# qwopqwop200/GPTQ-for-LLaMa

Hardware: NVIDIA H100
Metric: tokens/sec LLaMA-7B int4 g128 batch=1; matvec HBM GB/s vs 3.35 TB/s roofline (higher is better)
Workload: dtype f16

## Files before the change

### gptq-for-llama_b200/csrc/decode_mega.cu

```cuda
#include <cuda.h>
#include <cudaTypedefs.h>

#include "common.cuh"
#include "int4_core.cuh"
#include "kernels.h"

namespace gptq {
namespace {

using namespace int4;

constexpr int kTeams = 2;
constexpr int kTeamWarps = 8;
constexpr int kTeamThreads = kTeamWarps * 32;
constexpr int kConsumers = kTeams * kTeamThreads;
constexpr int kConsumerWarps = kTeams * kTeamWarps;
constexpr int kBlock = kConsumers + 32 * kTeams;
constexpr int kSlabCols = 256;
constexpr int kStageSteps = 4;
constexpr int kStepBytes = 4096;
constexpr int kScaleOff = kStageSteps * kStepBytes;
constexpr int kZeroOff = kScaleOff + 512;
constexpr int kStageBytes = 17 * 1024;
constexpr int kHD = 128;
// ... 55 lines not shown

struct MatDesc {
    const __half* sc;
    const uint32_t* qz;
    int gs_steps;
    int tmap;
    int chunk0;
};
struct LayerDesc {
    MatDesc qkv, o, gate, up, down;
    const __half* input_norm;
    const __half* post_norm;
    const int32_t* qkv_perm;
    const int32_t* o_perm;
    const int32_t* mlp_perm;
};
constexpr int kMaxTP = 8;
struct MegaParams {
    int n_layers, H, Hq, I, V, v0, v1, n_heads, max_seq, n_stages, lm_rows;
    int tp_size, tp_rank, tp_exchange;
    float eps, inv_base, scale;
    const __half* embed;
    const __half* final_norm;
    const __half* lm_head;
    const int32_t* tokens;
    const int32_t* positions;
    __half* k_cache;
    __half* v_cache;
    size_t layer_stride;
    __half* logits;
    int32_t* next_token;
    __half* resid[2];
    float* acc_qkv;
    float* acc_o;
    float* acc_g;
    float* acc_u;
    float* acc_d;
    float* part;
    float* rope_cs;
    unsigned long long* bar;
    float* acc_o_loc;
    float* acc_d_loc;
    float* acc_o_peer[kMaxTP];
    float* acc_d_peer[kMaxTP];
    __half* logits_peer[kMaxTP];
    unsigned long long* xbar_peer[kMaxTP];
    LayerDesc layers[kMaxLayers];
    CUtensorMap tmaps[6];
    int batch, xs_stride;
};

__device__ __forceinline__ void team_range(unsigned T, unsigned U, unsigned nb, int& a, int& b) {
    a = (int)((T * U) / nb);
    b = (int)(((T + 1) * U) / nb);
}
struct HeadTeams {
    int first, count;
};
__device__ __forceinline__ HeadTeams head_teams(int head, int n_heads, unsigned nb) {
    const int base = (int)nb / n_heads, rem = (int)nb % n_heads;
    HeadTeams h;
    h.first = head * base + min(head, rem);
    h.count = base + (head < rem ? 1 : 0);
    return h;
}
__device__ __forceinline__ void attn_range(unsigned T, int n_heads, unsigned nb, int upb, int& head, int& b0, int& b1) {
    const int base = (int)nb / n_heads, rem = (int)nb % n_heads;
    const int split = rem * (base + 1);
    int idx, cnt;
    if ((int)T < split) {
        head = (int)T / (base + 1);
        idx = (int)T - head * (base + 1);
        cnt = base + 1;
    } else {
        head = rem + ((int)T - split) / base;
        idx = ((int)T - split) % base;
        cnt = base;
// ... 18 lines not shown
    }
    const long long extra = (long long)nb - (long long)p.batch * p.n_heads;
    HeadTeams h;
    h.first = s * p.n_heads + (int)(extra * before / tot);
    h.count = (s + 1) * p.n_heads + (int)(extra * (before + mine) / tot) - h.first;
    return h;
}
__device__ __forceinline__ int team_seq(const MegaParams& p, unsigned T, unsigned nb, HeadTeams& st) {
    int s = 0;
#pragma unroll 1
    for (;; ++s) {
        st = seq_teams(p, s, nb);
        if ((int)T < st.first + st.count || s == p.batch - 1) return s;
    }
}
template <bool BATCH>
__device__ __forceinline__ int attn_work(const MegaParams& p, unsigned T, unsigned nb, int& pos, int& Tlen, int& head, int& b0, int& b1) {
    int s = 0;
    HeadTeams st{0, (int)nb};
    if constexpr (BATCH) {
        s = team_seq(p, T, nb, st);
        pos = step_pos(p, s);
    } else {
        pos = step_pos(p);
    }
    Tlen = pos + 1;
    const int upb = (Tlen + kKeysPerUnit - 1) / kKeysPerUnit;
    attn_range(T - st.first, p.n_heads, st.count, upb, head, b0, b1);
    return s;
}

__device__ __forceinline__ void team_sync(int team) { asm volatile("bar.sync %0, 256;" ::"r"(team + 1) : "memory"); }
__device__ __forceinline__ void cta_sync() { asm volatile("bar.sync 3, 512;" ::: "memory"); }

struct ProdRing {
    uint32_t ring, full, empty;
    int stage, use, nstages;
#ifdef GPTQ_TRACE
    long long blocked;
#endif
};
__device__ __forceinline__ uint32_t prod_acquire(ProdRing& r, uint32_t& bar) {
#ifdef GPTQ_TRACE
    const long long t0 = clock64();
#endif
    if (r.use > 0) mbar_wait_backoff(r.empty + r.stage * 8, (r.use - 1) & 1u);
#ifdef GPTQ_TRACE
    r.blocked += clock64() - t0;
#endif
    bar = r.full + r.stage * 8;
    return r.ring + r.stage * kStageBytes;
}
__device__ __forceinline__ void prod_advance(ProdRing& r) {
    if (++r.stage == r.nstages) {
        r.stage = 0;
        ++r.use;
    }
}

__device__ __forceinline__ void tma_load_3d(uint32_t dst, const CUtensorMap* tm, int c0, int c1, int c2, uint32_t bar) {
    asm volatile("cp.async.bulk.tensor.3d.shared::cluster.global.mbarrier::complete_tx::bytes [%0], [%1, {%2, %3, %4}], [%5];" ::"r"(dst), "l"(tm), "r"(c0),
                 "r"(c1), "r"(c2), "r"(bar)
                 : "memory");
}

template <int NM>
// ... 335 lines not shown
        a[1] = h2_as_u32(__hfma2(nibbles_to_h2<0x00f000f0u>(q), sixteenth, m64));
        a[2] = h2_as_u32(__hsub2(nibbles_to_h2<0x000f000fu>(q8), c1024));
        a[3] = h2_as_u32(__hfma2(nibbles_to_h2<0x00f000f0u>(q8), sixteenth, m64));
    }
}

template <bool FIRST>
__device__ __forceinline__ void step_mma(const uint4& q, const uint4& xf, float (&acc0)[4], float (&acc1)[4]) {
    uint32_t c0[4], c1[4], c2[4], c3[4];
    nibble_regs(q.x, c0);
    nibble_regs(q.y, c1);
    nibble_regs(q.z, c2);
    nibble_regs(q.w, c3);
    if (FIRST) {
        mma_16816_z(acc0, c0[0], c1[0], c0[1], c1[1], xf.x, xf.y);
        mma_16816_z(acc1, c2[0], c3[0], c2[1], c3[1], xf.x, xf.y);
    } else {
        mma_16816(acc0, c0[0], c1[0], c0[1], c1[1], xf.x, xf.y);
        mma_16816(acc1, c2[0], c3[0], c2[1], c3[1], xf.x, xf.y);
    }
    mma_16816(acc0, c0[2], c1[2], c0[3], c1[3], xf.z, xf.w);
    mma_16816(acc1, c2[2], c3[2], c2[3], c3[3], xf.z, xf.w);
}

enum XMode { X_FULL = 0, X_ATTN = 1, X_SWIGLU = 2 };

struct TeamCtx {
    int team, wt, lane, ttid;
    unsigned T, nb;
    __half* xseg;
    float* xsum_seg;
    uint8_t* scratch;
};

template <int NB>
__device__ __forceinline__ float merge_records(const MegaParams& p, const HeadTeams& ht, int d) {
    float M = -INFINITY, Ls = 0.f, O = 0.f;
#pragma unroll 1
    for (int ib = 0; ib < ht.count; ib += NB) {
        float mv[NB], lv[NB], ov[NB];
#pragma unroll
        for (int i = 0; i < NB; ++i) {
            const bool on = ib + i < ht.count;
            const float* rc = p.part + (size_t)(ht.first + (on ? ib + i : 0)) * kRec;
            const float m = ld_cg(rc), l = ld_cg(rc + 1), o = ld_cg(rc + 4 + d);
            mv[i] = on ? m : -INFINITY;
            lv[i] = on ? l : 0.f;
            ov[i] = on ? o : 0.f;
        }
        float Mb = M;
#pragma unroll
        for (int i = 0; i < NB; ++i) Mb = fmaxf(Mb, mv[i]);
        const float w0 = (M == -INFINITY) ? 0.f : expf(M - Mb);
        Ls *= w0;
        O *= w0;
#pragma unroll
        for (int i = 0; i < NB; ++i) {
            const float w = (mv[i] == -INFINITY) ? 0.f : expf(mv[i] - Mb);
            Ls = fmaf(lv[i], w, Ls);
            O = fmaf(ov[i], w, O);
        }
        M = Mb;
    }
    return O / Ls;
}

// ... 147 lines not shown
            const uint32_t o1 = h2_as_u32(__floats2half2_rn(swiglu(g0.z, a0.z), swiglu(g0.w, a0.w)));
            const uint32_t o2 = h2_as_u32(__floats2half2_rn(swiglu(g1.x, a1.x), swiglu(g1.y, a1.y)));
            const uint32_t o3 = h2_as_u32(__floats2half2_rn(swiglu(g1.z, a1.z), swiglu(g1.w, a1.w)));
            *reinterpret_cast<uint4*>(tc.xseg + (size_t)s * p.xs_stride + cs * 8) = perm8(o0, o1, o2, o3);
        }
    } else {
#pragma unroll 1
        for (int s = 0; s < B; ++s) {
            const HeadTeams st = seq_teams(p, s, tc.nb);
            __half* xseg = tc.xseg + (size_t)s * p.xs_stride;
            for (int e = tc.ttid; e < nfeat; e += kTeamThreads) {
                int k = k_of(e);
                if constexpr (ACT) {
                    if (perm != nullptr) k = perm[k];
                }
                const int head = k / kHD, d = k - head * kHD;
                HeadTeams ht = head_teams(head, p.n_heads, st.count);
                ht.first += st.first;
                __half hv = __float2half_rn(merge_records<12>(p, ht, d));
                const int j8 = e & 7;
                if (perm_scaled(j8)) hv = __hmul(hv, __float2half_rn(0.0625f));
                xseg[(e & ~7) + perm_pos(j8)] = hv;
            }
        }
    }
    team_sync(tc.team);
#pragma unroll 1
    for (int s = 0; s < B; ++s) compute_xsum(tc.xseg + (size_t)s * p.xs_stride, nun, tc.xsum_seg + s * (p.H / 32), tc.ttid, kTeamThreads);
    team_sync(tc.team);
}

template <int NM, int XMODE, bool ACT = false, bool BATCH = false>
__device__ void run_matvec(const MegaParams& p, ConsRing& ring, const TeamCtx& tc, int gs_steps, int K, int N, float* out0, float* out1, const __half* xs_full,
                           const float* xsum_full, const int32_t* perm = nullptr, float* const* peers = nullptr) {
    const int lane = tc.lane, g = lane >> 2, t = lane & 3;
    const int nk = K / 32, nslab = N / kSlabCols;
    int u, u_end;
    team_range(tc.T, (unsigned)(NM * nslab) * nk, tc.nb, u, u_end);
    const int cg = (g >> 1) | ((g & 1) << 2);
    const int col_l = 4 * cg + t;
    const uint32_t lane_a0 = (uint32_t)((tc.wt * 16 + t) * 128 + ((cg ^ t) * 16));
    const uint32_t lane_a1 = (uint32_t)((tc.wt * 16 + t) * 128 + ((cg ^ t ^ 4) * 16));
    const uint32_t lane_b = (uint32_t)((tc.wt * 4 + t) * 128 + ((cg ^ (4 * (tc.wt & 1) + t)) * 16));
    const uint32_t lane_s = (uint32_t)(kScaleOff + (tc.wt * 32 + col_l) * 2);
    const uint32_t lane_z = (uint32_t)(kZeroOff + (tc.wt * 4 + (cg >> 1)) * 4);
    const int zshift = (cg & 1) * 16 + t * 4;
    const float unit = kSubnormal ? 16777216.0f : 1.0f;
    const int B = p.batch;
    const int xsum_hi = BATCH ? (min(2 * t + 1, B - 1) - min(2 * t, B - 1)) * (p.H / 32) : 0;
    const int u_begin = u;
    if constexpr (XMODE != X_FULL) {
        if (u < u_end) {
#ifdef GPTQ_TRACE
            const long long stg0 = clock64();
#endif
            if constexpr (BATCH)
                stage_range_batch<XMODE, ACT>(p, tc, nk, u, u_end, perm);
            else
                stage_range<XMODE, ACT>(p, tc, nk, u, u_end, perm);
#ifdef GPTQ_TRACE
            if (g_mega_trace != nullptr && threadIdx.x == 0) g_mega_trace[blockIdx.x * 64 + 36 + XMODE] += (unsigned long long)(clock64() - stg0);
#endif
        }
    }

#pragma unroll 1
    while (u < u_end) {
// ... 70 lines not shown
                }
            } else {
                uint32_t sh, zw;
                asm volatile("ld.shared.u16 %0, [%1];" : "=r"(sh) : "r"(st + lane_s));
                asm volatile("ld.shared.u32 %0, [%1];" : "=r"(zw) : "r"(st + lane_z));
                const float a = (t & 2) ? ((t & 1) ? acc1[2] : acc1[0]) : ((t & 1) ? acc0[2] : acc0[0]);
                const float z = (float)(((zw >> zshift) & 15u) + 1u);
                tot = fmaf(__half2float(__ushort_as_half((unsigned short)sh)), fmaf(a, unit, -z * xs4), tot);
            }
            cons_release(ring, lane);
            xaddr += n * 64;
            xsum += n;
            left -= n;
            gpos += n;
            if (gpos == gs_steps) gpos = 0;
        }
        if constexpr (BATCH) {
            float* outq = (mi ? out1 : out0) + (slab_v - mi * nslab) * kSlabCols + tc.wt * 32 + 4 * cg;
#pragma unroll
            for (int j = 0; j < 2; ++j) {
                if (2 * t + j < B)
                    asm volatile("red.global.add.v4.f32 [%0], {%1, %2, %3, %4};" ::"l"(outq + (size_t)(2 * t + j) * N), "f"(totb[0][j]), "f"(totb[1][j]),
                                 "f"(totb[2][j]), "f"(totb[3][j])
                                 : "memory");
            }
        } else if (peers == nullptr) {
            asm volatile("red.global.add.f32 [%0], %1;" ::"l"(outp), "f"(tot) : "memory");
        } else {
            const size_t off = (size_t)(outp - out0);
            for (int q = 0; q < p.tp_size; ++q) asm volatile("red.relaxed.sys.global.add.f32 [%0], %1;" ::"l"(peers[q] + off), "f"(tot) : "memory");
        }
        u += nseg;
    }
}

template <bool BATCH>
__device__ void run_attention(const MegaParams& p, ConsRing& ring, const TeamCtx& tc, int layer) {
    int pos, Tlen, head, b0, b_end;
    const int seq = attn_work<BATCH>(p, tc.T, tc.nb, pos, Tlen, head, b0, b_end);
    float* red_o = reinterpret_cast<float*>(tc.scratch);
    float* red_ml = reinterpret_cast<float*>(tc.scratch + 4096);
    float* q_s = reinterpret_cast<float*>(tc.scratch);
    __half* knew = reinterpret_cast<__half*>(tc.scratch + 512);
    __half* vnew = knew + kHD;
    const int ttid = tc.ttid, lane = tc.lane, grp = ttid >> 3, j = ttid & 7;
    const int ub_new = pos / kKeysPerUnit;
    __half* kc_l = p.k_cache + layer * p.layer_stride;
    __half* vc_l = p.v_cache + layer * p.layer_stride;
    float* rec = p.part + (size_t)tc.T * kRec;
    if (b0 >= b_end) {
        if (ttid < kHD) rec[4 + ttid] = 0.f;
        if (ttid == 0) {
            rec[0] = -INFINITY;
            rec[1] = 0.f;
        }
        return;
    }
    {
        const int nseg = b_end - b0;
        const bool owns_new = (ub_new >= b0 && ub_new < b_end);
        team_sync(tc.team);
        if (ttid < kHD) {
            const int i = ttid & 63;
            const bool hi = ttid >= 64;
            const float c = ld_cg(p.rope_cs + seq * kHD + i), s = ld_cg(p.rope_cs + seq * kHD + 64 + i);
            const float* aq = p.acc_qkv + (size_t)seq * 3 * p.Hq + head * kHD;
            const float qx = __half2float(__float2half_rn(ld_cg(aq + i))), qy = __half2float(__float2half_rn(ld_cg(aq + i + 64)));
            const float qr = hi ? __fadd_rn(__fmul_rn(qx, s), __fmul_rn(qy, c)) : __fsub_rn(__fmul_rn(qx, c), __fmul_rn(qy, s));
            q_s[ttid] = __half2float(__float2half_rn(qr));
            if (owns_new) {
                const float* ak = aq + p.Hq;
                const float* av = aq + 2 * p.Hq;
                const float kx = __half2float(__float2half_rn(ld_cg(ak + i))), ky = __half2float(__float2half_rn(ld_cg(ak + i + 64)));
                const float kr = hi ? __fadd_rn(__fmul_rn(kx, s), __fmul_rn(ky, c)) : __fsub_rn(__fmul_rn(kx, c), __fmul_rn(ky, s));
                const __half kh = __float2half_rn(kr), vh = __float2half_rn(ld_cg(av + ttid));
                knew[ttid] = kh;
                vnew[ttid] = vh;
                const size_t off = ((size_t)(seq * p.n_heads + head) * p.max_seq + pos) * kHD + ttid;
                kc_l[off] = kh;
                vc_l[off] = vh;
            }
        }
        team_sync(tc.team);
        float qr[16];
#pragma unroll
        for (int d = 0; d < 8; ++d) {
            qr[d] = q_s[8 * j + d];
            qr[8 + d] = q_s[64 + 8 * j + d];
        }
        float mloc = -INFINITY, lloc = 0.f, o[16];
#pragma unroll
        for (int d = 0; d < 16; ++d) o[d] = 0.f;
#pragma unroll 1
        for (int b = b0; b < b0 + nseg; ++b) {
            const uint32_t st = cons_wait(ring);
            if (b == ub_new) {
                team_sync(tc.team);
                const int row = pos - b * kKeysPerUnit;
// ... 55 lines not shown
            mloc = mn;
        }
        if (lane < 8) {
            if (lane == 0) {
                red_ml[tc.wt * 2] = mloc;
                red_ml[tc.wt * 2 + 1] = lloc;
            }
#pragma unroll
            for (int d = 0; d < 8; ++d) {
                red_o[tc.wt * kHD + 8 * lane + d] = o[d];
                red_o[tc.wt * kHD + 64 + 8 * lane + d] = o[8 + d];
            }
        }
        team_sync(tc.team);
        if (ttid < kHD) {
            float M = -INFINITY;
#pragma unroll
            for (int w = 0; w < kTeamWarps; ++w) M = fmaxf(M, red_ml[w * 2]);
            float L = 0.f, O = 0.f;
#pragma unroll
            for (int w = 0; w < kTeamWarps; ++w) {
                const float mw = red_ml[w * 2];
                const float wgt = (mw == -INFINITY) ? 0.f : expf(mw - M);
                L = fmaf(red_ml[w * 2 + 1], wgt, L);
                O = fmaf(red_o[w * kHD + ttid], wgt, O);
            }
            rec[4 + ttid] = O;
            if (ttid == 0) {
                rec[0] = M;
                rec[1] = L;
            }
        }
    }
}

__device__ void run_lm_head(const MegaParams& p, ConsRing& ring, const TeamCtx& tc, const __half* xs_plain) {
    const int R = p.lm_rows, H = p.H, nch = H / 8;
    int u, u_end;
    const int nloc = p.v1 - p.v0;
    team_range(tc.T, (unsigned)((nloc + R - 1) / R), tc.nb, u, u_end);
    float* part_s = reinterpret_cast<float*>(tc.scratch);
    float xr[4][8];
#pragma unroll
    for (int i = 0; i < 4; ++i) {
        const int c = tc.ttid + i * kTeamThreads;
        if (c < nch) {
            const uint4 v = *reinterpret_cast<const uint4*>(xs_plain + c * 8);
            const uint32_t w[4] = {v.x, v.y, v.z, v.w};
#pragma unroll
            for (int e = 0; e < 4; ++e) {
                const float2 f = __half22float2(u32_as_h2(w[e]));
                xr[i][2 * e] = f.x;
                xr[i][2 * e + 1] = f.y;
            }
        } else {
#pragma unroll
            for (int e = 0; e < 8; ++e) xr[i][e] = 0.f;
        }
    }
    int buf = 0;
#pragma unroll 1
    for (; u < u_end; ++u) {
        const int nrows = min(R, nloc - u * R);
        const uint32_t st = cons_wait(ring);
        float* ps = part_s + buf * (R * kTeamWarps);
#pragma unroll 1
// ... 178 lines not shown
    ConsRing ring;
    ring.ring = smem_u32(smem_raw) + tc.team * ring_bytes;
    ring.full = smem_u32(&bars_s[tc.team][0]);
    ring.tile = ring.ring;
    ring.bar = ring.full;
    ring.parity = 0;
    ring.left = p.n_stages;
    ring.nstages = p.n_stages;
#ifdef GPTQ_TRACE
    ring.waited = 0;
    ring.stages = 0;
#endif

    unsigned long long gen;
    {
        unsigned long long v;
        asm volatile("ld.acquire.gpu.global.u64 %0, [%1];" : "=l"(v) : "l"(p.bar + 1) : "memory");
        gen = v;
    }
    unsigned long long xgen = 0;
    if (p.tp_size > 1) asm volatile("ld.acquire.sys.global.u64 %0, [%1];" : "=l"(xgen) : "l"(p.xbar_peer[p.tp_rank] + 32 * kMaxTP) : "memory");
    auto sync_all_ranks = [&](float* loc, float* const* peers) {
        if (p.tp_size == 1) {
            grid_barrier(p.bar, gen);
        } else {
            if (p.tp_exchange && loc != nullptr) {
                grid_barrier(p.bar, gen);
                tp_exchange(p, loc, peers, p.H);
            }
            tp_barrier(p, xgen);
        }
    };

    if constexpr (BATCH) {
        if (blockIdx.x == 0 && tid < 64 * nbat) {
            const int s = tid >> 6, i = tid & 63;
            const float f = expf((float)i * p.inv_base) * (float)step_pos(p, s);
            p.rope_cs[s * kHD + i] = cosf(f);
            p.rope_cs[s * kHD + 64 + i] = sinf(f);
        }
    } else if (blockIdx.x == 0 && tid < 64) {
        const float f = expf((float)tid * p.inv_base) * (float)step_pos(p);
        p.rope_cs[tid] = cosf(f);
        p.rope_cs[64 + tid] = sinf(f);
    }

    const int token = min(max(p.tokens[0], 0), p.V - 1);
    const __half* resid_src = p.embed + (size_t)token * p.H;
    const float* resid_acc = nullptr;
    int cur = 1;
    auto stage_norms = [&](bool plain, const __half* src, const float* acc, const __half* norm_w, __half* resid_out, const int32_t* perm) {
#pragma unroll 1
        for (int s = 0; s < nbat; ++s) {
            const __half* src_s = acc != nullptr ? src + (size_t)s * p.H : p.embed + (size_t)min(max(p.tokens[s], 0), p.V - 1) * p.H;
            const float* acc_s = acc != nullptr ? acc + (size_t)s * p.H : nullptr;
            __half* out_s = resid_out != nullptr ? resid_out + (size_t)s * p.H : nullptr;
            if (plain)
                stage_norm<false, true>(p, src_s, acc_s, norm_w, out_s, xs + (size_t)s * p.xs_stride, xsum + s * (p.H / 32), tmp, red_s, nullptr);
            else
                stage_norm<ACT, false>(p, src_s, acc_s, norm_w, out_s, xs + (size_t)s * p.xs_stride, xsum + s * (p.H / 32), tmp, red_s, perm);
        }
    };
#pragma unroll 1
    for (int l = 0; l < p.n_layers; ++l) {
        const LayerDesc& L = p.layers[l];
        MTRACE(l * 12 + 0);
        if constexpr (BATCH)
            stage_norms(false, resid_src, resid_acc, L.input_norm, p.resid[cur ^ 1], L.qkv_perm);
        else
            stage_norm<ACT, false>(p, resid_src, resid_acc, L.input_norm, p.resid[cur ^ 1], xs, xsum, tmp, red_s, L.qkv_perm);
        MTRACE(l * 12 + 1);
        cur ^= 1;
        zero_slice(p.acc_g, nbat * p.I);
        zero_slice(p.acc_u, nbat * p.I);
        {
            OPTRACE_BEGIN(ring);
            run_matvec<1, X_FULL, false, BATCH>(p, ring, tc, L.qkv.gs_steps, p.H, 3 * p.Hq, p.acc_qkv, nullptr, xs, xsum);
            OPTRACE_END(ring, l, 0);
        }
        MTRACE(l * 12 + 2);
        grid_barrier(p.bar, gen);
        MTRACE(l * 12 + 3);
        zero_slice(p.acc_d, nbat * p.H);
        {
            OPTRACE_BEGIN(ring);
            run_attention<BATCH>(p, ring, tc, l);
            OPTRACE_END(ring, l, 1);
        }
        MTRACE(l * 12 + 4);
        grid_barrier(p.bar, gen);
        MTRACE(l * 12 + 5);
        zero_slice(p.acc_qkv, nbat * 3 * p.Hq);
        {
            OPTRACE_BEGIN(ring);
            if constexpr (BATCH)
                run_matvec<1, X_ATTN, ACT, true>(p, ring, tc, L.o.gs_steps, p.Hq, p.H, p.acc_o, nullptr, xs, xsum, L.o_perm);
            else
                run_matvec<1, X_ATTN, ACT>(p, ring, tc, L.o.gs_steps, p.Hq, p.H, p.tp_exchange ? p.acc_o_loc : p.acc_o, nullptr, xs, xsum, L.o_perm, (p.tp_size > 1 && !p.tp_exchange) ? p.acc_o_peer : nullptr);
            OPTRACE_END(ring, l, 2);
        }
        MTRACE(l * 12 + 6);
        sync_all_ranks(p.acc_o_loc, p.acc_o_peer);
        MTRACE(l * 12 + 7);
        if constexpr (BATCH)
            stage_norms(false, p.resid[cur], p.acc_o, L.post_norm, p.resid[cur ^ 1], L.mlp_perm);
        else
            stage_norm<ACT, false>(p, p.resid[cur], p.acc_o, L.post_norm, p.resid[cur ^ 1], xs, xsum, tmp, red_s, L.mlp_perm);
        cur ^= 1;
        MTRACE(l * 12 + 8);
        {
            OPTRACE_BEGIN(ring);
            run_matvec<2, X_FULL, false, BATCH>(p, ring, tc, L.gate.gs_steps, p.H, p.I, p.acc_g, p.acc_u, xs, xsum);
            OPTRACE_END(ring, l, 3);
        }
        MTRACE(l * 12 + 9);
        grid_barrier(p.bar, gen);
        zero_slice(p.acc_o, nbat * p.H);
        MTRACE(l * 12 + 10);
        {
            OPTRACE_BEGIN(ring);
            if constexpr (BATCH)
                run_matvec<1, X_SWIGLU, false, true>(p, ring, tc, L.down.gs_steps, p.I, p.H, p.acc_d, nullptr, xs, xsum);
            else
                run_matvec<1, X_SWIGLU>(p, ring, tc, L.down.gs_steps, p.I, p.H, p.tp_exchange ? p.acc_d_loc : p.acc_d, nullptr, xs, xsum, nullptr, (p.tp_size > 1 && !p.tp_exchange) ? p.acc_d_peer : nullptr);
            OPTRACE_END(ring, l, 4);
        }
        MTRACE(l * 12 + 11);
        sync_all_ranks(p.acc_d_loc, p.acc_d_peer);
        resid_src = p.resid[cur];
        resid_acc = p.acc_d;
    }
    if constexpr (BATCH)
        stage_norms(true, resid_src, resid_acc, p.final_norm, nullptr, nullptr);
    else
        stage_norm<false, true>(p, resid_src, resid_acc, p.final_norm, nullptr, xs, xsum, tmp, red_s, nullptr);
    zero_slice(p.acc_g, nbat * p.I);
    zero_slice(p.acc_u, nbat * p.I);
    if constexpr (BATCH)
        run_lm_head_batch(p, ring, tc, xs);
    else
        run_lm_head(p, ring, tc, xs);
    sync_all_ranks(nullptr, nullptr);
    zero_slice(p.acc_d, nbat * p.H);
    if constexpr (BATCH) {
        if (blockIdx.x == 0 && tid == 0) p.bar[1] = gen;
        if ((int)blockIdx.x < nbat && p.next_token != nullptr) argmax_row(p.logits + (size_t)blockIdx.x * p.V, p.V, p.next_token + blockIdx.x);
    } else if (blockIdx.x == 0) {
        if (tid == 0) {
            p.bar[1] = gen;
            if (p.tp_size > 1) p.xbar_peer[p.tp_rank][32 * kMaxTP] = xgen;
        }
        if (p.next_token != nullptr) {
            float best = -INFINITY;
            int idx = 0x7fffffff;
            for (int i = tid; i < p.V; i += kConsumers) {
                const float v = __half2float(ld_cg_h(p.logits + i));
                if (v > best || (v == best && i < idx)) {
                    best = v;
                    idx = i;
                }
            }
            __shared__ float sv[kConsumerWarps];
            __shared__ int si[kConsumerWarps];
#pragma unroll
            for (int o = 16; o > 0; o >>= 1) {
                const float ov = __shfl_xor_sync(0xffffffffu, best, o);
                const int oi = __shfl_xor_sync(0xffffffffu, idx, o);
                if (ov > best || (ov == best && oi < idx)) {
                    best = ov;
                    idx = oi;
                }
            }
            if (lane == 0) {
                sv[warp] = best;
                si[warp] = idx;
            }
// ... 73 lines not shown
        if (tp.size < 1 || tp.size > kMaxTP || tp.rank < 0 || tp.rank >= tp.size) return false;
        if (tp.vocab_begin < 0 || tp.vocab_end > m.vocab || tp.vocab_begin >= tp.vocab_end) return false;
        for (int q = 0; q < tp.size; ++q)
            if (q != tp.rank && (tp.peer_scratch[q] == nullptr || tp.peer_logits[q] == nullptr)) return false;
    } else if (m.n_heads * m.head_dim != m.hidden) {
        return false;
    }
    for (int l = 0; l < m.n_layers; ++l) {
        const gptq_llama_layer& ly = m.layers[l];
        const gptq_qweight* ws[5] = {&ly.qkv, &ly.o, &ly.gate, &ly.up, &ly.down};
        for (const gptq_qweight* w : ws) {
            if (w->bits != 4 || w->groupsize <= 0 || w->groupsize % 32) return false;
            if ((reinterpret_cast<uintptr_t>(w->qweight) & 15) || (reinterpret_cast<uintptr_t>(w->scales) & 15) || (reinterpret_cast<uintptr_t>(w->qzeros) & 15))
                return false;
        }
        if (ly.gate.groupsize != ly.up.groupsize) return false;
    }
    if ((reinterpret_cast<uintptr_t>(m.lm_head) & 15) || (reinterpret_cast<uintptr_t>(st.k_cache) & 15) || (reinterpret_cast<uintptr_t>(st.v_cache) & 15)) return false;
    int dev = 0, sms = 0, smem_optin = 0;
    cudaFuncAttributes fa;
    if (cudaGetDevice(&dev) == cudaSuccess && cudaDeviceGetAttribute(&sms, cudaDevAttrMultiProcessorCount, dev) == cudaSuccess &&
        cudaDeviceGetAttribute(&smem_optin, cudaDevAttrMaxSharedMemoryPerBlockOptin, dev) == cudaSuccess &&
        cudaFuncGetAttributes(&fa, llama_decode_mega_kernel<false, false>) == cudaSuccess) {
        MegaPlan pl;
        if (sms * kTeams > 1024 || !mega_plan(m, st.batch, sms, (size_t)smem_optin, fa.sharedSizeBytes, pl)) return false;
    }
    return true;
}

size_t mega_scratch_bytes(const gptq_llama_model& m, int batch, int max_seq) {
    (void)max_seq;
    const size_t max_teams = 1024;
    const size_t B = (size_t)batch;
    return al256(B * m.hidden * 2) * 2 + al256(B * 3 * m.hidden * 4) + al256(B * m.hidden * 4) * 2 + al256(B * m.intermediate * 4) * 2 +
           al256(max_teams * kRec * 4) + al256(B * 128 * 4) + 256 + (kMaxTP + 1) * 256 + al256((size_t)m.hidden * 4) * 2;
}

cudaError_t launch_decode_mega(const gptq_llama_model& m, const gptq_llama_state& st, uint8_t* scratch, cudaStream_t stream) {
    static_assert(sizeof(MegaParams) < 32000, "kernel parameter space");
    int dev = 0, sms = 0, smem_optin = 0;
    if (cudaGetDevice(&dev) != cudaSuccess || cudaDeviceGetAttribute(&sms, cudaDevAttrMultiProcessorCount, dev) != cudaSuccess ||
        cudaDeviceGetAttribute(&smem_optin, cudaDevAttrMaxSharedMemoryPerBlockOptin, dev) != cudaSuccess)
        return cudaErrorInvalidDevice;
    bool any_perm = false;
    for (int l = 0; l < m.n_layers; ++l) any_perm = any_perm || m.layers[l].qkv_perm != nullptr || m.layers[l].o_perm != nullptr || m.layers[l].mlp_perm != nullptr;
    const int B = st.batch;
    auto kernel = B > 1 ? (any_perm ? llama_decode_mega_kernel<true, true> : llama_decode_mega_kernel<false, true>)
                        : (any_perm ? llama_decode_mega_kernel<true, false> : llama_decode_mega_kernel<false, false>);
    cudaFuncAttributes fa;
    if (cudaFuncGetAttributes(&fa, kernel) != cudaSuccess) return cudaErrorInvalidDeviceFunction;
    MegaPlan pl;
    if (sms * kTeams > 1024 || !mega_plan(m, B, sms, (size_t)smem_optin, fa.sharedSizeBytes, pl)) return cudaErrorInvalidConfiguration;

    MegaParams p{};
    p.n_layers = m.n_layers; p.H = m.hidden; p.Hq = m.n_heads * m.head_dim; p.I = m.intermediate; p.V = m.vocab; p.n_heads = m.n_heads;
    p.v0 = st.tp != nullptr ? st.tp->vocab_begin : 0;
    p.v1 = st.tp != nullptr ? st.tp->vocab_end : m.vocab;
    p.max_seq = st.max_seq;
    p.n_stages = pl.n_stages;
    p.lm_rows = pl.lm_rows;
    p.eps = m.rms_eps;
    p.inv_base = (float)(-2.0 * log((double)m.rope_base) / (double)m.head_dim);
    p.scale = 1.0f / sqrtf((float)m.head_dim);
    p.embed = reinterpret_cast<const __half*>(m.embed);
    p.final_norm = reinterpret_cast<const __half*>(m.final_norm);
    p.lm_head = reinterpret_cast<const __half*>(m.lm_head);
    p.tokens = st.tokens;
    p.positions = st.positions;
    p.k_cache = reinterpret_cast<__half*>(st.k_cache);
    p.v_cache = reinterpret_cast<__half*>(st.v_cache);
    p.layer_stride = (size_t)B * m.n_heads * st.max_seq * m.head_dim;
    p.logits = reinterpret_cast<__half*>(st.logits);
    p.next_token = st.next_tokens;
    p.batch = B;
    p.xs_stride = xs_stride(m.hidden);
    size_t off = 0;
    auto take = [&](size_t bytes) {
        uint8_t* q = scratch + off;
        off += al256(bytes);
        return q;
    };
    p.resid[0] = reinterpret_cast<__half*>(take((size_t)B * m.hidden * 2));
    p.resid[1] = reinterpret_cast<__half*>(take((size_t)B * m.hidden * 2));
    p.acc_o = reinterpret_cast<float*>(take((size_t)B * m.hidden * 4));
    p.acc_d = reinterpret_cast<float*>(take((size_t)B * m.hidden * 4));
    unsigned long long* xbar = reinterpret_cast<unsigned long long*>(take((kMaxTP + 1) * 256));
    const gptq_llama_tp* tp = st.tp;
    p.tp_size = tp != nullptr ? tp->size : 1;
    p.tp_rank = tp != nullptr ? tp->rank : 0;
    p.tp_exchange = (tp != nullptr && tp->size > 1) ? (tp->reduce_mode == 0 ? (tp->size > 4) : (tp->reduce_mode == 2)) : 0;
    for (int q = 0; q < p.tp_size; ++q) {
        uint8_t* base = (tp != nullptr && q != tp->rank) ? reinterpret_cast<uint8_t*>(tp->peer_scratch[q]) : scratch;
        p.acc_o_peer[q] = reinterpret_cast<float*>(base + (reinterpret_cast<uint8_t*>(p.acc_o) - scratch));
        p.acc_d_peer[q] = reinterpret_cast<float*>(base + (reinterpret_cast<uint8_t*>(p.acc_d) - scratch));
        p.xbar_peer[q] = reinterpret_cast<unsigned long long*>(base + (reinterpret_cast<uint8_t*>(xbar) - scratch));
        p.logits_peer[q] = reinterpret_cast<__half*>((tp != nullptr && q != tp->rank) ? tp->peer_logits[q] : st.logits);
    }
    p.acc_o_loc = reinterpret_cast<float*>(take((size_t)m.hidden * 4));
    p.acc_d_loc = reinterpret_cast<float*>(take((size_t)m.hidden * 4));
    p.acc_qkv = reinterpret_cast<float*>(take((size_t)B * 3 * p.Hq * 4));
    p.acc_g = reinterpret_cast<float*>(take((size_t)B * m.intermediate * 4));
    p.acc_u = reinterpret_cast<float*>(take((size_t)B * m.intermediate * 4));
    p.part = reinterpret_cast<float*>(take((size_t)1024 * kRec * 4));
    p.rope_cs = reinterpret_cast<float*>(take((size_t)B * 128 * 4));
    p.bar = reinterpret_cast<unsigned long long*>(take(256));
    const int classN[3] = {3 * m.n_heads * m.head_dim, m.hidden, m.intermediate};
    uintptr_t base[3] = {UINTPTR_MAX, UINTPTR_MAX, UINTPTR_MAX}, top[3] = {0, 0, 0};
    int rows_max[3] = {0, 0, 0};
    auto visit = [&](const gptq_qweight& w, int c) {
        const uintptr_t a = reinterpret_cast<uintptr_t>(w.qweight);
        base[c] = a < base[c] ? a : base[c];
        top[c] = a > top[c] ? a : top[c];
        rows_max[c] = max(rows_max[c], w.K / 8);
    };
    for (int l = 0; l < m.n_layers; ++l) {
        const gptq_llama_layer& ly = m.layers[l];
        visit(ly.qkv, 0); visit(ly.o, 1); visit(ly.down, 1); visit(ly.gate, 2); visit(ly.up, 2);
    }
    for (int c = 0; c < 3; ++c) {
        if ((base[c] & 127) != 0) return cudaErrorInvalidConfiguration;
        const uint64_t chunks = (uint64_t)(top[c] - base[c]) / 128 + (uint64_t)classN[c] / 32;
        if (chunks >= (1ull << 31)) return cudaErrorInvalidConfiguration;
        for (int v = 0; v < 2; ++v)
            if (!encode_weight_map(&p.tmaps[3 * v + c], reinterpret_cast<const void*>(base[c]), rows_max[c], chunks, classN[c], v == 0 ? 4 * kStageSteps : 4))
                return cudaErrorNotSupported;
    }
    bool act = false;
    for (int l = 0; l < m.n_layers; ++l) {
        const gptq_llama_layer& ly = m.layers[l];
        bool aligned = true;
        auto md = [&](const gptq_qweight& w, int c) {
            MatDesc d;
            d.sc = reinterpret_cast<const __half*>(w.scales);
            d.qz = reinterpret_cast<const uint32_t*>(w.qzeros);
            d.gs_steps = w.groupsize / 32;
            d.tmap = c;
            const uintptr_t delta = reinterpret_cast<uintptr_t>(w.qweight) - base[c];
            aligned = aligned && (delta % 128 == 0);
// ... 43 lines not shown
```

Baseline: 397.4.

## Replace grid barriers with per-slab dataflow counters and double-buffered accumulators

Removes three grid-wide barriers per layer. In their place, teams bump release counters as they finish qkv and gate/up slabs and attention heads, and consumers spin with acquire loads on only the counters for the inputs they need. The o/down accumulators are double-buffered by layer parity so zeroing can be deferred without racing. RoPE cos/sin is now computed inline in attention rather than precomputed, and named barriers let the sibling team reuse the shared x segment. This adds polling traffic and a risk of deadlock or counter-target mismatch in exchange for less idle time at barriers.

```diff
diff --git a/gptq-for-llama_b200/csrc/decode_mega.cu b/gptq-for-llama_b200/csrc/decode_mega.cu
--- a/gptq-for-llama_b200/csrc/decode_mega.cu
+++ b/gptq-for-llama_b200/csrc/decode_mega.cu
@@ -111,17 +111,20 @@
     int32_t* next_token;
     __half* resid[2];
     float* acc_qkv;
-    float* acc_o;
+    float* acc_o[2];
     float* acc_g;
     float* acc_u;
-    float* acc_d;
+    float* acc_d[2];
     float* part;
-    float* rope_cs;
     unsigned long long* bar;
+    unsigned* cnt_qkv;
+    unsigned* cnt_gu;
+    unsigned* cnt_head;
+    int n_cnt;
     float* acc_o_loc;
     float* acc_d_loc;
-    float* acc_o_peer[kMaxTP];
-    float* acc_d_peer[kMaxTP];
+    float* acc_o_peer[2][kMaxTP];
+    float* acc_d_peer[2][kMaxTP];
     __half* logits_peer[kMaxTP];
     unsigned long long* xbar_peer[kMaxTP];
     LayerDesc layers[kMaxLayers];
@@ -206,6 +209,8 @@
 
 __device__ __forceinline__ void team_sync(int team) { asm volatile("bar.sync %0, 256;" ::"r"(team + 1) : "memory"); }
 __device__ __forceinline__ void cta_sync() { asm volatile("bar.sync 3, 512;" ::: "memory"); }
+__device__ __forceinline__ void sibling_done_with_xs(int team) { asm volatile("bar.arrive %0, 512;" ::"r"(4 + (team ^ 1)) : "memory"); }
+__device__ __forceinline__ void wait_xs_free(int team) { asm volatile("bar.sync %0, 512;" ::"r"(4 + team) : "memory"); }
 
 struct ProdRing {
     uint32_t ring, full, empty;
@@ -607,6 +612,44 @@
     float* xsum_seg;
     uint8_t* scratch;
 };
+
+__device__ __forceinline__ void team_signal(const TeamCtx& tc, unsigned* cnt, unsigned n) {
+    team_sync(tc.team);
+    if (tc.ttid == 0) asm volatile("red.release.gpu.global.add.u32 [%0], %1;" ::"l"(cnt), "r"(n) : "memory");
+}
+template <class F>
+__device__ __forceinline__ void team_wait(const TeamCtx& tc, int n, F&& want) {
+    if (tc.wt == 0) {
+        for (int i = tc.lane; i < n; i += 32) {
+            const unsigned* c;
+            unsigned target, v;
+            want(i, c, target);
+            do {
+                asm volatile("ld.acquire.gpu.global.u32 %0, [%1];" : "=r"(v) : "l"(c) : "memory");
+            } while (v < target);
+        }
+    }
+    team_sync(tc.team);
+}
+struct Span {
+    int a0, na, nb;
+    __device__ __forceinline__ int n() const { return na + nb; }
+    __device__ __forceinline__ int at(int i) const { return i < na ? a0 + i : i - na; }
+};
+__device__ __forceinline__ Span input_span(int u, int u1, int nk, int per) {
+    const int nun = u1 - u;
+    if (nun >= nk) return Span{0, nk / per, 0};
+    const int a0 = u % nk, a1 = min(nk, a0 + nun), b1 = nun - (a1 - a0);
+    return Span{a0 / per, a1 > a0 ? (a1 - 1) / per - a0 / per + 1 : 0, b1 > 0 ? (b1 - 1) / per + 1 : 0};
+}
+template <bool BATCH>
+__device__ __forceinline__ unsigned head_records(const MegaParams& p, int head, unsigned nb) {
+    if constexpr (!BATCH) return (unsigned)head_teams(head, p.n_heads, nb).count;
+    unsigned n = 0;
+#pragma unroll 1
+    for (int s = 0; s < p.batch; ++s) n += (unsigned)head_teams(head, p.n_heads, seq_teams(p, s, nb).count).count;
+    return n;
+}
 
 template <int NB>
 __device__ __forceinline__ float merge_records(const MegaParams& p, const HeadTeams& ht, int d) {
@@ -820,7 +863,7 @@
 
 template <int NM, int XMODE, bool ACT = false, bool BATCH = false>
 __device__ void run_matvec(const MegaParams& p, ConsRing& ring, const TeamCtx& tc, int gs_steps, int K, int N, float* out0, float* out1, const __half* xs_full,
-                           const float* xsum_full, const int32_t* perm = nullptr, float* const* peers = nullptr) {
+                           const float* xsum_full, const int32_t* perm = nullptr, float* const* peers = nullptr, unsigned* done = nullptr) {
     const int lane = tc.lane, g = lane >> 2, t = lane & 3;
     const int nk = K / 32, nslab = N / kSlabCols;
     int u, u_end;
@@ -957,6 +1000,18 @@
         }
         u += nseg;
     }
+    if (done != nullptr && u_begin < u_end) {
+        team_sync(tc.team);
+        if (tc.ttid == 0) {
+            fence_acq_rel_gpu();
+#pragma unroll 1
+            for (int v = u_begin; v < u_end;) {
+                const int n = min(nk - v % nk, u_end - v);
+                asm volatile("red.relaxed.gpu.global.add.u32 [%0], %1;" ::"l"(done + v / nk), "r"((unsigned)n) : "memory");
+                v += n;
+            }
+        }
+    }
 }
 
 template <bool BATCH>
@@ -973,12 +1028,20 @@
     __half* kc_l = p.k_cache + layer * p.layer_stride;
     __half* vc_l = p.v_cache + layer * p.layer_stride;
     float* rec = p.part + (size_t)tc.T * kRec;
+    if (b0 < b_end) {
+        team_wait(tc, 3, [&](int i, const unsigned*& c, unsigned& target) {
+            c = p.cnt_qkv + (i * p.Hq + head * kHD) / kSlabCols;
+            target = (unsigned)(layer + 1) * (unsigned)(p.H / 32);
+        });
+    }
+    MTRACE(layer * 12 + 3);
     if (b0 >= b_end) {
         if (ttid < kHD) rec[4 + ttid] = 0.f;
         if (ttid == 0) {
             rec[0] = -INFINITY;
             rec[1] = 0.f;
         }
+        team_signal(tc, p.cnt_head + head, 1);
         return;
     }
     {
@@ -988,7 +1051,8 @@
         if (ttid < kHD) {
             const int i = ttid & 63;
             const bool hi = ttid >= 64;
-            const float c = ld_cg(p.rope_cs + seq * kHD + i), s = ld_cg(p.rope_cs + seq * kHD + 64 + i);
+            const float f = expf((float)i * p.inv_base) * (float)pos;
+            const float c = cosf(f), s = sinf(f);
             const float* aq = p.acc_qkv + (size_t)seq * 3 * p.Hq + head * kHD;
             const float qx = __half2float(__float2half_rn(ld_cg(aq + i))), qy = __half2float(__float2half_rn(ld_cg(aq + i + 64)));
             const float qr = hi ? __fadd_rn(__fmul_rn(qx, s), __fmul_rn(qy, c)) : __fsub_rn(__fmul_rn(qx, c), __fmul_rn(qy, s));
@@ -1110,6 +1174,7 @@
             }
         }
     }
+    team_signal(tc, p.cnt_head + head, 1);
 }
 
 __device__ void run_lm_head(const MegaParams& p, ConsRing& ring, const TeamCtx& tc, const __half* xs_plain) {
@@ -1354,19 +1419,6 @@
         }
     };
 
-    if constexpr (BATCH) {
-        if (blockIdx.x == 0 && tid < 64 * nbat) {
-            const int s = tid >> 6, i = tid & 63;
-            const float f = expf((float)i * p.inv_base) * (float)step_pos(p, s);
-            p.rope_cs[s * kHD + i] = cosf(f);
-            p.rope_cs[s * kHD + 64 + i] = sinf(f);
-        }
-    } else if (blockIdx.x == 0 && tid < 64) {
-        const float f = expf((float)tid * p.inv_base) * (float)step_pos(p);
-        p.rope_cs[tid] = cosf(f);
-        p.rope_cs[64 + tid] = sinf(f);
-    }
-
     const int token = min(max(p.tokens[0], 0), p.V - 1);
     const __half* resid_src = p.embed + (size_t)token * p.H;
     const float* resid_acc = nullptr;
@@ -1395,75 +1447,102 @@
         cur ^= 1;
         zero_slice(p.acc_g, nbat * p.I);
         zero_slice(p.acc_u, nbat * p.I);
+        if (l > 0) zero_slice(p.acc_o[(l - 1) & 1], nbat * p.H);
+        const unsigned k_done = (unsigned)(l + 1) * (unsigned)(p.H / 32);
         {
             OPTRACE_BEGIN(ring);
-            run_matvec<1, X_FULL, false, BATCH>(p, ring, tc, L.qkv.gs_steps, p.H, 3 * p.Hq, p.acc_qkv, nullptr, xs, xsum);
+            run_matvec<1, X_FULL, false, BATCH>(p, ring, tc, L.qkv.gs_steps, p.H, 3 * p.Hq, p.acc_qkv, nullptr, xs, xsum, nullptr, nullptr, p.cnt_qkv);
             OPTRACE_END(ring, l, 0);
         }
+        sibling_done_with_xs(tc.team);
         MTRACE(l * 12 + 2);
-        grid_barrier(p.bar, gen);
-        MTRACE(l * 12 + 3);
-        zero_slice(p.acc_d, nbat * p.H);
         {
             OPTRACE_BEGIN(ring);
             run_attention<BATCH>(p, ring, tc, l);
             OPTRACE_END(ring, l, 1);
         }
         MTRACE(l * 12 + 4);
-        grid_barrier(p.bar, gen);
+        {
+            int u, u1;
+            team_range(tc.T, (unsigned)(p.H / kSlabCols) * (p.Hq / 32), tc.nb, u, u1);
+            const Span sp = (ACT && L.o_perm != nullptr) ? Span{0, p.n_heads, 0} : input_span(u, u1, p.Hq / 32, kHD / 32);
+            team_wait(tc, sp.n(), [&](int i, const unsigned*& c, unsigned& target) {
+                const int h = sp.at(i);
+                c = p.cnt_head + h;
+                target = (unsigned)(l + 1) * head_records<BATCH>(p, h, tc.nb);
+            });
+        }
+        wait_xs_free(tc.team);
         MTRACE(l * 12 + 5);
-        zero_slice(p.acc_qkv, nbat * 3 * p.Hq);
         {
             OPTRACE_BEGIN(ring);
             if constexpr (BATCH)
-                run_matvec<1, X_ATTN, ACT, true>(p, ring, tc, L.o.gs_steps, p.Hq, p.H, p.acc_o, nullptr, xs, xsum, L.o_perm);
+                run_matvec<1, X_ATTN, ACT, true>(p, ring, tc, L.o.gs_steps, p.Hq, p.H, p.acc_o[l & 1], nullptr, xs, xsum, L.o_perm);
             else
-                run_matvec<1, X_ATTN, ACT>(p, ring, tc, L.o.gs_steps, p.Hq, p.H, p.tp_exchange ? p.acc_o_loc : p.acc_o, nullptr, xs, xsum, L.o_perm, (p.tp_size > 1 && !p.tp_exchange) ? p.acc_o_peer : nullptr);
+                run_matvec<1, X_ATTN, ACT>(p, ring, tc, L.o.gs_steps, p.Hq, p.H, p.tp_exchange ? p.acc_o_loc : p.acc_o[l & 1], nullptr, xs, xsum, L.o_perm,
+                                           (p.tp_size > 1 && !p.tp_exchange) ? p.acc_o_peer[l & 1] : nullptr);
             OPTRACE_END(ring, l, 2);
         }
         MTRACE(l * 12 + 6);
-        sync_all_ranks(p.acc_o_loc, p.acc_o_peer);
+        sync_all_ranks(p.acc_o_loc, p.acc_o_peer[l & 1]);
         MTRACE(l * 12 + 7);
         if constexpr (BATCH)
-            stage_norms(false, p.resid[cur], p.acc_o, L.post_norm, p.resid[cur ^ 1], L.mlp_perm);
+            stage_norms(false, p.resid[cur], p.acc_o[l & 1], L.post_norm, p.resid[cur ^ 1], L.mlp_perm);
         else
-            stage_norm<ACT, false>(p, p.resid[cur], p.acc_o, L.post_norm, p.resid[cur ^ 1], xs, xsum, tmp, red_s, L.mlp_perm);
+            stage_norm<ACT, false>(p, p.resid[cur], p.acc_o[l & 1], L.post_norm, p.resid[cur ^ 1], xs, xsum, tmp, red_s, L.mlp_perm);
         cur ^= 1;
+        zero_slice(p.acc_qkv, nbat * 3 * p.Hq);
+        if (l > 0) zero_slice(p.acc_d[(l - 1) & 1], nbat * p.H);
         MTRACE(l * 12 + 8);
         {
             OPTRACE_BEGIN(ring);
-            run_matvec<2, X_FULL, false, BATCH>(p, ring, tc, L.gate.gs_steps, p.H, p.I, p.acc_g, p.acc_u, xs, xsum);
+            run_matvec<2, X_FULL, false, BATCH>(p, ring, tc, L.gate.gs_steps, p.H, p.I, p.acc_g, p.acc_u, xs, xsum, nullptr, nullptr, p.cnt_gu);
             OPTRACE_END(ring, l, 3);
         }
+        sibling_done_with_xs(tc.team);
         MTRACE(l * 12 + 9);
-        grid_barrier(p.bar, gen);
-        zero_slice(p.acc_o, nbat * p.H);
+        {
+            int u, u1;
+            team_range(tc.T, (unsigned)(p.H / kSlabCols) * (p.I / 32), tc.nb, u, u1);
+            const Span sp = input_span(u, u1, p.I / 32, kSlabCols / 32);
+            const int nsl = p.I / kSlabCols;
+            team_wait(tc, 2 * sp.n(), [&](int i, const unsigned*& c, unsigned& target) {
+                const int m = i >= sp.n() ? 1 : 0;
+                c = p.cnt_gu + m * nsl + sp.at(i - m * sp.n());
+                target = k_done;
+            });
+        }
+        wait_xs_free(tc.team);
         MTRACE(l * 12 + 10);
         {
             OPTRACE_BEGIN(ring);
             if constexpr (BATCH)
-                run_matvec<1, X_SWIGLU, false, true>(p, ring, tc, L.down.gs_steps, p.I, p.H, p.acc_d, nullptr, xs, xsum);
+                run_matvec<1, X_SWIGLU, false, true>(p, ring, tc, L.down.gs_steps, p.I, p.H, p.acc_d[l & 1], nullptr, xs, xsum);
             else
-                run_matvec<1, X_SWIGLU>(p, ring, tc, L.down.gs_steps, p.I, p.H, p.tp_exchange ? p.acc_d_loc : p.acc_d, nullptr, xs, xsum, nullptr, (p.tp_size > 1 && !p.tp_exchange) ? p.acc_d_peer : nullptr);
+                run_matvec<1, X_SWIGLU>(p, ring, tc, L.down.gs_steps, p.I, p.H, p.tp_exchange ? p.acc_d_loc : p.acc_d[l & 1], nullptr, xs, xsum, nullptr,
+                                        (p.tp_size > 1 && !p.tp_exchange) ? p.acc_d_peer[l & 1] : nullptr);
             OPTRACE_END(ring, l, 4);
         }
         MTRACE(l * 12 + 11);
-        sync_all_ranks(p.acc_d_loc, p.acc_d_peer);
+        sync_all_ranks(p.acc_d_loc, p.acc_d_peer[l & 1]);
         resid_src = p.resid[cur];
-        resid_acc = p.acc_d;
-    }
+        resid_acc = p.acc_d[l & 1];
+    }
+    const int last = (p.n_layers - 1) & 1;
     if constexpr (BATCH)
         stage_norms(true, resid_src, resid_acc, p.final_norm, nullptr, nullptr);
     else
         stage_norm<false, true>(p, resid_src, resid_acc, p.final_norm, nullptr, xs, xsum, tmp, red_s, nullptr);
     zero_slice(p.acc_g, nbat * p.I);
     zero_slice(p.acc_u, nbat * p.I);
+    zero_slice(p.acc_o[last], nbat * p.H);
     if constexpr (BATCH)
         run_lm_head_batch(p, ring, tc, xs);
     else
         run_lm_head(p, ring, tc, xs);
     sync_all_ranks(nullptr, nullptr);
-    zero_slice(p.acc_d, nbat * p.H);
+    zero_slice(p.acc_d[last], nbat * p.H);
+    for (int i = blockIdx.x * kConsumers + tid; i < p.n_cnt; i += gridDim.x * kConsumers) p.cnt_qkv[i] = 0u;
     if constexpr (BATCH) {
         if (blockIdx.x == 0 && tid == 0) p.bar[1] = gen;
         if ((int)blockIdx.x < nbat && p.next_token != nullptr) argmax_row(p.logits + (size_t)blockIdx.x * p.V, p.V, p.next_token + blockIdx.x);
@@ -1603,8 +1682,9 @@
     (void)max_seq;
     const size_t max_teams = 1024;
     const size_t B = (size_t)batch;
-    return al256(B * m.hidden * 2) * 2 + al256(B * 3 * m.hidden * 4) + al256(B * m.hidden * 4) * 2 + al256(B * m.intermediate * 4) * 2 +
-           al256(max_teams * kRec * 4) + al256(B * 128 * 4) + 256 + (kMaxTP + 1) * 256 + al256((size_t)m.hidden * 4) * 2;
+    const size_t counters = (size_t)(3 * m.hidden + 2 * m.intermediate) / kSlabCols + (size_t)m.hidden / kHD;
+    return al256(B * m.hidden * 2) * 2 + al256(B * 3 * m.hidden * 4) + al256(B * m.hidden * 4) * 4 + al256(B * m.intermediate * 4) * 2 +
+           al256(max_teams * kRec * 4) + 256 + al256(counters * 4) + (kMaxTP + 1) * 256 + al256((size_t)m.hidden * 4) * 2;
 }
 
 cudaError_t launch_decode_mega(const gptq_llama_model& m, const gptq_llama_state& st, uint8_t* scratch, cudaStream_t stream) {
@@ -1653,28 +1733,36 @@
     };
     p.resid[0] = reinterpret_cast<__half*>(take((size_t)B * m.hidden * 2));
     p.resid[1] = reinterpret_cast<__half*>(take((size_t)B * m.hidden * 2));
-    p.acc_o = reinterpret_cast<float*>(take((size_t)B * m.hidden * 4));
-    p.acc_d = reinterpret_cast<float*>(take((size_t)B * m.hidden * 4));
+    p.acc_o[0] = reinterpret_cast<float*>(take((size_t)B * m.hidden * 4));
+    p.acc_d[0] = reinterpret_cast<float*>(take((size_t)B * m.hidden * 4));
     unsigned long long* xbar = reinterpret_cast<unsigned long long*>(take((kMaxTP + 1) * 256));
+    p.acc_o_loc = reinterpret_cast<float*>(take((size_t)m.hidden * 4));
+    p.acc_d_loc = reinterpret_cast<float*>(take((size_t)m.hidden * 4));
+    p.acc_o[1] = reinterpret_cast<float*>(take((size_t)B * m.hidden * 4));
+    p.acc_d[1] = reinterpret_cast<float*>(take((size_t)B * m.hidden * 4));
     const gptq_llama_tp* tp = st.tp;
     p.tp_size = tp != nullptr ? tp->size : 1;
     p.tp_rank = tp != nullptr ? tp->rank : 0;
     p.tp_exchange = (tp != nullptr && tp->size > 1) ? (tp->reduce_mode == 0 ? (tp->size > 4) : (tp->reduce_mode == 2)) : 0;
     for (int q = 0; q < p.tp_size; ++q) {
         uint8_t* base = (tp != nullptr && q != tp->rank) ? reinterpret_cast<uint8_t*>(tp->peer_scratch[q]) : scratch;
-        p.acc_o_peer[q] = reinterpret_cast<float*>(base + (reinterpret_cast<uint8_t*>(p.acc_o) - scratch));
-        p.acc_d_peer[q] = reinterpret_cast<float*>(base + (reinterpret_cast<uint8_t*>(p.acc_d) - scratch));
+        for (int par = 0; par < 2; ++par) {
+            p.acc_o_peer[par][q] = reinterpret_cast<float*>(base + (reinterpret_cast<uint8_t*>(p.acc_o[par]) - scratch));
+            p.acc_d_peer[par][q] = reinterpret_cast<float*>(base + (reinterpret_cast<uint8_t*>(p.acc_d[par]) - scratch));
+        }
         p.xbar_peer[q] = reinterpret_cast<unsigned long long*>(base + (reinterpret_cast<uint8_t*>(xbar) - scratch));
         p.logits_peer[q] = reinterpret_cast<__half*>((tp != nullptr && q != tp->rank) ? tp->peer_logits[q] : st.logits);
     }
-    p.acc_o_loc = reinterpret_cast<float*>(take((size_t)m.hidden * 4));
-    p.acc_d_loc = reinterpret_cast<float*>(take((size_t)m.hidden * 4));
     p.acc_qkv = reinterpret_cast<float*>(take((size_t)B * 3 * p.Hq * 4));
     p.acc_g = reinterpret_cast<float*>(take((size_t)B * m.intermediate * 4));
     p.acc_u = reinterpret_cast<float*>(take((size_t)B * m.intermediate * 4));
     p.part = reinterpret_cast<float*>(take((size_t)1024 * kRec * 4));
-    p.rope_cs = reinterpret_cast<float*>(take((size_t)B * 128 * 4));
     p.bar = reinterpret_cast<unsigned long long*>(take(256));
+    const int n_qkv = 3 * p.Hq / kSlabCols, n_gu = 2 * m.intermediate / kSlabCols;
+    p.n_cnt = n_qkv + n_gu + m.n_heads;
+    p.cnt_qkv = reinterpret_cast<unsigned*>(take((size_t)p.n_cnt * 4));
+    p.cnt_gu = p.cnt_qkv + n_qkv;
+    p.cnt_head = p.cnt_gu + n_gu;
     const int classN[3] = {3 * m.n_heads * m.head_dim, m.hidden, m.intermediate};
     uintptr_t base[3] = {UINTPTR_MAX, UINTPTR_MAX, UINTPTR_MAX}, top[3] = {0, 0, 0};
     int rows_max[3] = {0, 0, 0};
```

After: 410.7 (median of 6 runs). +3.3%, better.
